# acbull/pyHGT

Measured on AMD Instinct MI355X. Metric: HGTConv forward edges/sec, higher is better.
Workload: dtype f32 (typed linears and relation transforms as 3-term fp16 hi/lo MFMA with power-of-two row scales, fp32 accumulate)

## Files before the change

include/hgt_hip.h:

```cpp
#ifndef HGT_HIP_H_
#define HGT_HIP_H_

#include <stddef.h>
#include <stdint.h>

#ifdef __cplusplus
extern "C" {
#endif

#define HGT_ABI_VERSION 8

#define HGT_OK 0
#define HGT_ERR_INVALID_ARG (-1)
#define HGT_ERR_UNSUPPORTED (-2)
#define HGT_ERR_WORKSPACE (-3)
#define HGT_ERR_TOO_LARGE (-4)
#define HGT_ERR_LAUNCH (-5)

#define HGT_RTE_LEN 240

const char* hgt_strerror(int code);
int hgt_abi_version(void);
#define HGT_FEATURE_LAB_KERNELS 1
#define HGT_FEATURE_DETERMINISTIC_TRAINING 2
// ... 76 lines not shown
                             void* stream);
int hgt_linear_update_f16x3(const float* agg, int64_t ld_agg, const int32_t* rows, const int32_t* group_off,
                            int32_t n_groups, int64_t n_rows, int32_t k, int32_t n_out, const void* w_split,
                            const float* bias, int64_t b_group_stride, const float* x_skip, int64_t ld_skip,
                            const float* skip, const float* ln_w, const float* ln_b, int32_t use_norm, float* out,
                            void* stream);
int hgt_zero_rows(const int32_t* rows, const int32_t* range, int32_t d, float* out, void* stream);

int hgt_relation_pack(const float* relation_att, const float* relation_msg, const float* relation_pri,
                      int32_t n_relations, int32_t n_heads, int32_t n_heads_layout, int32_t d_k, int32_t dk_pad,
                      float* att_t, float* msg_p, void* stream);

int hgt_edge_logits(const void* plan, int64_t n_nodes, int64_t n_edges, int32_t n_types, int32_t n_relations,
                    int32_t n_heads, int32_t dk_pad, const float* Q, const float* K, const float* rte_k,
                    const float* att_t, float* logits, void* stream);
int hgt_edge_logits_mfma(const void* plan, int64_t n_nodes, int64_t n_edges, int32_t n_types, int32_t n_relations,
                         int32_t n_heads, int32_t dk_pad, const float* Q, const float* K, const float* rte_k,
                         const float* att_t, const void* att_frag, int32_t frag_f16, float* logits, void* stream);
int hgt_relation_kside_bytes(int32_t n_relations, int32_t n_heads, int32_t dk_pad, uint64_t* out_host);
int hgt_relation_kside_pack(const float* att_t, int32_t n_relations, int32_t n_heads, int32_t dk_pad, void* att_kside, void* stream);
int hgt_edge_logits_kside(const void* plan, int64_t n_nodes, int64_t n_edges, int32_t n_types, int32_t n_relations,
                          int32_t n_heads, int32_t dk_pad, const float* Q, const float* K, const float* rte_k,
                          const float* att_t, const void* att_kside, int32_t frag_f16, float* logits, void* stream);
int hgt_kside_image_map(int32_t n_blocks, int32_t* image_map, int32_t* b_col, int32_t* c_out);
int hgt_edge_logits_range(const void* plan, int64_t n_nodes, int64_t n_edges, int32_t n_types, int32_t n_relations,
                          int32_t n_heads, int32_t dk_pad, const float* Q, const float* K, const float* rte_k,
                          const float* att_t, const void* att_frag, int32_t frag_f16, float* logits, int32_t item_begin,
                          int32_t item_end, void* stream);
int hgt_edge_softmax(const void* plan, int64_t n_nodes, int64_t n_edges, int32_t n_types, int32_t n_relations,
                     int32_t n_heads, float* logits_att, void* stream);
int hgt_edge_aggregate(const void* plan, int64_t n_nodes, int64_t n_edges, int32_t n_types, int32_t n_relations,
                       int32_t n_heads, int32_t dk_pad, const float* logits, const float* V, const float* rte_v,
                       const float* msg_p, const void* msg_frag, float* agg, int64_t n_q_rows, int32_t apply_gelu,
                       void* hub_ws, void* stream);
int hgt_edge_aggregate_items_bytes(int64_t n_edges, int32_t n_heads, int32_t dk_pad, uint64_t* out_host);
int hgt_edge_aggregate_items(const void* plan, int64_t n_nodes, int64_t n_edges, int32_t n_types, int32_t n_relations,
                             int32_t n_heads, int32_t dk_pad, const float* logits, const float* V, const float* rte_v,
                             const void* msg_frag, int32_t frag_f16, float* agg, int64_t n_q_rows, int32_t apply_gelu,
                             void* scratch, uint64_t scratch_bytes, void* stream);
int hgt_edge_aggregate_items_update(const void* plan, int64_t n_nodes, int64_t n_edges, int32_t n_types, int32_t n_relations,
                                    int32_t n_heads, int32_t dk_pad, const float* logits, const float* V, const float* rte_v,
                                    const void* msg_frag, int32_t frag_f16, int64_t n_q_rows, void* scratch, uint64_t scratch_bytes,
                                    const int32_t* rows, const int32_t* group_off, int32_t n_groups, const void* w_a_split,
                                    const float* b_a, const float* x_skip, int64_t ld_skip, const float* skip, const float* ln_w,
                                    const float* ln_b, int32_t use_norm, int32_t n_out, float* out, void* stream);
int hgt_edge_single_pass_items(const void* plan, int64_t n_nodes, int64_t n_edges, int32_t n_types, int32_t n_relations,
// ... 174 lines not shown
    int32_t stage;
    const int32_t* proj_rows;
    const int32_t* proj_off;
    int64_t proj_n;
    void* prepared;
    uint64_t prepared_bytes;
    int32_t prepared_valid;
    int32_t plan_no_hubs;
    int32_t flags;
    int32_t slice_index;
    int32_t slice_count;
    int64_t q_begin, q_end;
    int32_t item_begin, item_end;
    const void* proj_c24;
    int64_t proj_c24_row0;
} hgt_conv_args;

#define HGT_FLAG_NO_FUSED_UPDATE 1
#define HGT_FLAG_VALU_AGGREGATE  2
#define HGT_FLAG_MFMA_LOGITS     4
#define HGT_FLAG_VALU_LOGITS     8
#define HGT_FLAG_KSIDE_LOGITS 65536
#define HGT_FLAG_NO_KSIDE_LOGITS 131072
#define HGT_FLAG_ITEM_AGGREGATE 16
#define HGT_FLAG_NO_ITEM_AGGREGATE 32
#define HGT_FLAG_FUSED_ANY_SIZE 64
#define HGT_FLAG_SINGLE_PASS 256
#define HGT_FLAG_XS_GEMM_ALWAYS 1024
#define HGT_FLAG_XS_GEMM_NEVER 2048
#define HGT_FLAG_NO_TILE_GEMM 4096
#define HGT_FLAG_NO_MERGE_UPDATE 8192
#define HGT_FLAG_NO_COOP_EDGE 16384
#define HGT_FLAG_COOP_EDGE_ALWAYS 32768
#define HGT_FLAG_RING_AGGREGATE 512
#define HGT_FLAG_DETERMINISTIC_HUBS 128

#define HGT_N_PHASE_EVENTS 7

int hgt_conv_workspace_bytes(int64_t n_nodes, int64_t n_edges, int32_t in_dim, int32_t out_dim,
                             int32_t n_types, int32_t n_relations, int32_t n_heads, int32_t use_rte,
                             uint64_t* out_host);
int hgt_conv_workspace_bytes_ex(int64_t n_nodes, int64_t n_edges, int32_t in_dim, int32_t out_dim,
                                int32_t n_types, int32_t n_relations, int32_t n_heads, int32_t use_rte, int32_t options,
                                uint64_t* out_host);
int hgt_conv_prepared_bytes(int32_t in_dim, int32_t out_dim, int32_t n_types, int32_t n_relations, int32_t n_heads,
                            int32_t use_rte, uint64_t* out_host);
// ... 132 lines not shown
```

pyhgt_amd/_lib.py:

```python
import ctypes as C
import os

_HERE = os.path.dirname(os.path.abspath(__file__))
LIB_PATH = os.environ.get("HGT_LIB_PATH", os.path.join(_HERE, "lib", "libhgt_hip.so"))

HGT_RTE_LEN = 240
HGT_N_PHASE_EVENTS = 7
HGT_FLAG_NO_FUSED_UPDATE = 1
HGT_FLAG_VALU_AGGREGATE = 2
HGT_FLAG_MFMA_LOGITS = 4
HGT_FLAG_VALU_LOGITS = 8
HGT_FLAG_ITEM_AGGREGATE = 16
HGT_FLAG_NO_ITEM_AGGREGATE = 32
HGT_FLAG_FUSED_ANY_SIZE = 64
HGT_FLAG_DETERMINISTIC_HUBS = 128
HGT_FLAG_SINGLE_PASS = 256
HGT_FLAG_RING_AGGREGATE = 512
HGT_FLAG_XS_GEMM_ALWAYS = 1024
HGT_FLAG_XS_GEMM_NEVER = 2048
HGT_FLAG_NO_TILE_GEMM = 4096
HGT_FLAG_NO_MERGE_UPDATE = 8192
HGT_FLAG_NO_COOP_EDGE = 16384
HGT_FLAG_COOP_EDGE_ALWAYS = 32768
HGT_FLAG_KSIDE_LOGITS = 65536
HGT_FLAG_NO_KSIDE_LOGITS = 131072
HGT_LINEAR_FORCE_XS = 0x100
HGT_LINEAR_NO_XS = 0x200
HGT_LINEAR_NO_TILE = 0x400
HGT_LINEAR_TANH = 0x1000
HGT_FEATURE_LAB_KERNELS = 1
HGT_FEATURE_DETERMINISTIC_TRAINING = 2
HGT_STACK_MAX_PIECES = 256
HGT_SAMPLER_MAX_TYPES = 16
HGT_SAMPLER_MAX_TRIPLES = 48
HGT_SAMPLER_MAX_NUMBER = 1024
HGT_SAMPLER_HUB_DEG = 512
HGT_SAMPLER_TIME_NONE = -2 ** 31
HGT_SAMPLER_MAX_BATCH = 64


class HgtLayout(C.Structure):
    _fields_ = [("d_k", C.c_int32), ("dk_pad", C.c_int32), ("d_pad", C.c_int32), ("vec", C.c_int32), ("heads", C.c_int32)]


class HgtPlanSizes(C.Structure):
    _fields_ = [("plan_bytes", C.c_uint64), ("tmp_bytes", C.c_uint64), ("max_items", C.c_int64), ("n_bins", C.c_int64)]


# ... 65 lines not shown
    "hgt_plan_build": (C.c_int, [_vp, _i64, _i64, _vp, _vp, _vp, _i64, _i64, _i64, _i32, _i32, _vp, _u64, _vp, _u64, _vp]),
    "hgt_plan_from_sorted": (C.c_int, [_vp, _vp, _vp, _vp, _vp, _i64, _i64, _i64, _i32, _i32, _vp, _u64, _vp, _u64, _vp]),
    "hgt_typed_linear": (C.c_int, [_vp, _i64, _vp, _vp, _i32, _i64, _i32, _i32, _vp, _i64, _vp, _i64, _vp, _vp, _vp,
                                   _i32, _i32, _i32, _i32, _vp]),
    "hgt_split_weights_bytes": (C.c_int, [_i32, _i32, _i32, C.POINTER(_u64)]),
    "hgt_split_weights": (C.c_int, [_vp, _i64, _i32, _i32, _i32, _vp, _vp]),
    "hgt_typed_linear_bf16x3": (C.c_int, [_vp, _i64, _vp, _vp, _i32, _i64, _i32, _i32, _vp, _vp, _i64, _vp, _vp, _vp,
                                          _i32, _i32, _i32, _vp]),
    "hgt_linear_update_bf16x3": (C.c_int, [_vp, _i64, _vp, _vp, _i32, _i64, _i32, _i32, _vp, _vp, _i64, _vp, _i64, _vp, _vp, _vp,
                                           _i32, _vp, _vp]),
    "hgt_split_weights_f16": (C.c_int, [_vp, _i64, _i32, _i32, _i32, _vp, _vp]),
    "hgt_typed_linear_xs_schedule": (C.c_int, [_vp, _i32, _i64, _i32, _i32, _vp, _i64, C.POINTER(_i64)]),
    "hgt_typed_linear_f16x3": (C.c_int, [_vp, _i64, _vp, _vp, _i32, _i64, _i32, _i32, _vp, _vp, _i64, _vp, _vp, _vp,
                                         _i32, _i32, _i32, _vp]),
    "hgt_linear_update_f16x3": (C.c_int, [_vp, _i64, _vp, _vp, _i32, _i64, _i32, _i32, _vp, _vp, _i64, _vp, _i64, _vp, _vp, _vp,
                                          _i32, _vp, _vp]),
    "hgt_zero_rows": (C.c_int, [_vp, _vp, _i32, _vp, _vp]),
    "hgt_relation_pack": (C.c_int, [_vp, _vp, _vp, _i32, _i32, _i32, _i32, _i32, _vp, _vp, _vp]),
    "hgt_edge_logits": (C.c_int, [_vp, _i64, _i64, _i32, _i32, _i32, _i32, _vp, _vp, _vp, _vp, _vp, _vp]),
    "hgt_edge_logits_mfma": (C.c_int, [_vp, _i64, _i64, _i32, _i32, _i32, _i32, _vp, _vp, _vp, _vp, _vp, _i32, _vp, _vp]),
    "hgt_relation_kside_bytes": (C.c_int, [_i32, _i32, _i32, C.POINTER(_u64)]),
    "hgt_relation_kside_pack": (C.c_int, [_vp, _i32, _i32, _i32, _vp, _vp]),
    "hgt_edge_logits_kside": (C.c_int, [_vp, _i64, _i64, _i32, _i32, _i32, _i32, _vp, _vp, _vp, _vp, _vp, _i32, _vp, _vp]),
    "hgt_kside_image_map": (C.c_int, [_i32, _vp, _vp, _vp]),
    "hgt_edge_logits_range": (C.c_int, [_vp, _i64, _i64, _i32, _i32, _i32, _i32, _vp, _vp, _vp, _vp, _vp, _i32, _vp, _i32, _i32, _vp]),
    "hgt_edge_aggregate_update_range": (C.c_int, [_vp, _i64, _i64, _i32, _i32, _i32, _i32, _vp, _vp, _vp, _vp, _vp, _vp, _i64, _vp, _vp, _vp,
                                                  _vp, _vp, _vp, _i64, _vp, _vp, _vp, _i32, _i32, _vp, _vp, _i64, _i64, _i32, _i32]),
    "hgt_hub_workspace_bytes_ex": (C.c_int, [_i64, _i32, _i32, _i32, _i32, C.POINTER(_u64)]),
    "hgt_edge_aggregate_ex": (C.c_int, [_vp, _i64, _i64, _i32, _i32, _i32, _i32, _vp, _vp, _vp, _vp, _vp, _i32, _vp, _i64, _i32, _vp, _i32, _vp]),
    "hgt_edge_logits_slice": (C.c_int, [_vp, _i64, _i64, _i32, _i32, _i32, _i32, _vp, _vp, _vp, _vp, _vp, _i32, _i32, _vp]),
    "hgt_edge_aggregate_slice": (C.c_int, [_vp, _i64, _i64, _i32, _i32, _i32, _i32, _vp, _vp, _vp, _vp, _vp, _vp, _i64, _i32, _vp,
                                           _i32, _i32, _vp, _i32, _i32, _vp]),
    "hgt_edge_aggregate_slice_ex": (C.c_int, [_vp, _i64, _i64, _i32, _i32, _i32, _i32, _vp, _vp, _vp, _vp, _vp, _vp, _i64, _i32, _vp,
                                              _i32, _i32, _vp, _i32, _i32, _i32, _vp]),
    "hgt_edge_softmax": (C.c_int, [_vp, _i64, _i64, _i32, _i32, _i32, _vp, _vp]),
    "hgt_edge_aggregate": (C.c_int, [_vp, _i64, _i64, _i32, _i32, _i32, _i32, _vp, _vp, _vp, _vp, _vp, _vp, _i64, _i32, _vp, _vp]),
    "hgt_edge_aggregate_f16x3": (C.c_int, [_vp, _i64, _i64, _i32, _i32, _i32, _i32, _vp, _vp, _vp, _vp, _vp, _vp, _i64, _i32, _vp, _vp]),
    "hgt_relation_frag_pack_f16": (C.c_int, [_vp, _i32, _i32, _i32, _vp, _vp]),
    "hgt_edge_aggregate_items_bytes": (C.c_int, [_i64, _i32, _i32, C.POINTER(_u64)]),
    "hgt_edge_spmm_items": (C.c_int, [_vp, _i64, _i64, _i32, _i32, _i32, _i32, _vp, _vp, _vp, _vp, _vp, _i64, _i64, _vp, _u64, _vp]),
    "hgt_edge_aggregate_items_update": (C.c_int, [_vp, _i64, _i64, _i32, _i32, _i32, _i32, _vp, _vp, _vp, _vp, _i32, _i64, _vp, _u64, _vp, _vp, _i32,
                                                  _vp, _vp, _vp, _i64, _vp, _vp, _vp, _i32, _i32, _vp, _vp]),
    "hgt_edge_aggregate_items": (C.c_int, [_vp, _i64, _i64, _i32, _i32, _i32, _i32, _vp, _vp, _vp, _vp, _i32, _vp, _i64, _i32, _vp, _u64, _vp]),
    "hgt_edge_single_pass_items": (C.c_int, [_vp, _i64, _i64, _i32, _i32, _i32, _i32, _vp, _vp, _vp, _vp, _vp, _vp, _vp, _i32, _vp, _i64, _i32,
                                             _vp, _u64, _vp]),
    "hgt_plan_header_to_host": (C.c_int, [_vp, _vp, _vp]),
    "hgt_relation_frag_bytes": (C.c_int, [_i32, _i32, _i32, C.POINTER(_u64)]),
# ... 119 lines not shown
```

pyhgt_amd/csrc/hgt_api.hip:

```cpp
#include "hgt_common.h"

#ifndef HGT_FUSED_MIN_NODES
#define HGT_FUSED_MIN_NODES 16384
#endif
#ifndef HGT_ITEM_AGG_MAX_NODES
#define HGT_ITEM_AGG_MAX_NODES 65536
#endif
#ifndef HGT_ITEM_AGG_DEFAULT_NODES
#define HGT_ITEM_AGG_DEFAULT_NODES 65536
#endif

int hgt_edge_logits_kside_items(const void* plan, int64_t N, int64_t E, int32_t T, int32_t R, int32_t H, int32_t dk_pad, const float* Q,
                                const float* K, const float* rte_k, const void* att_kside, float* logits, int item_lo, int item_hi, void* stream);

namespace {

struct ConvWorkspace {
    uint64_t off_q, off_k, off_v, off_logits, off_agg, off_trans, off_att_t, off_msg_p, off_msg_f, off_att_f, off_att_k, off_hub;
    uint64_t off_rte_lin, off_rte_k, off_rte_v, off_rte_rows, off_rte_off, off_ws_qkv, off_ws_a, off_ws_rte, off_off2, off_pending, off_state, off_zitems, zitems_bytes, total;
    void drop_item_scratch() { zitems_bytes = 0; total = off_zitems; }
};

static ConvWorkspace conv_workspace(int64_t N, int64_t NQ, int64_t E, int in_dim, int out_dim, int T, int R, int , int use_rte,
                                    const hgt_layout& lay, bool item_scratch = true, bool det_hubs = false) {
    const int H = lay.heads;
    ConvWorkspace w;
    uint64_t o = 0;
    auto take = [&](uint64_t bytes) { uint64_t r = o; o = hgt_align_up(o + bytes, 256); return r; };
    const uint64_t dp = (uint64_t)lay.d_pad;
    w.off_q = take((uint64_t)NQ * dp * 4);
    w.off_k = take((uint64_t)N * dp * 4);
    w.off_v = take((uint64_t)N * dp * 4);
    w.off_logits = take((uint64_t)E * H * 4);
    w.off_agg = take((uint64_t)NQ * dp * 4);
    w.off_trans = take((uint64_t)NQ * out_dim * 4);
    w.off_att_t = take((uint64_t)R * H * lay.dk_pad * lay.dk_pad * 4);
// ... 62 lines not shown
    hgt_relation_kside_bytes(R, H, lay.dk_pad, &b);
    p.off_att_k = take(b);
    hgt_split_weights_bytes(T, in_dim, 3 * lay.d_pad, &b);
    p.off_ws_qkv = take(b);
    hgt_split_weights_bytes(T, lay.d_pad, out_dim, &b);
    p.off_ws_upd = take(b);
    p.off_rte_k = take(use_rte ? (uint64_t)T * HGT_RTE_LEN * lay.d_pad * 4 : 0);
    p.off_rte_v = take(use_rte ? (uint64_t)T * HGT_RTE_LEN * lay.d_pad * 4 : 0);
    p.total = o;
    return p;
}

__global__ void k_rte_row_lists(int T, int32_t* __restrict__ rows, int32_t* __restrict__ off) {
    const int i = blockIdx.x * blockDim.x + threadIdx.x;
    if (i < T * HGT_RTE_LEN) rows[i] = i % HGT_RTE_LEN;
    if (i <= T) off[i] = i * HGT_RTE_LEN;
}

enum LogitsForm { LOGITS_VALU, LOGITS_MFMA, LOGITS_SLICE, LOGITS_RANGE, LOGITS_KSIDE };
enum AggForm { AGG_SINGLE_PASS, AGG_FUSED, AGG_ITEMS_UPDATE, AGG_ITEMS, AGG_SLICE, AGG_SUBTILE };
enum UpdateForm { UPDATE_IN_AGGREGATION, UPDATE_LINEAR_FUSED, UPDATE_LINEAR_NODE, UPDATE_DENSE };
struct ConvRoute {
    LogitsForm logits;
    bool kside_range;
    bool mfma_logits;
    AggForm agg[5];
    int n_agg;
    UpdateForm update;
};

struct Conv {
    const hgt_conv_args* a;
    hipStream_t stream;
    hgt_layout lay;
    ConvWorkspace w;
    PreparedLayout pl;
    hgt_plan_rows pr;
    int64_t N, E, NQ;
    int T, R, H, din, dout, dp, dkp, stage, fmode, sl_lo, sl_hi, sl_more;
    bool f16, split, dense, det_hubs, no_unknown_rows, have_frags, have_kside, mfma_agg;
    decltype(&hgt_split_weights) split_weights;
    bool fresh;
    bool wa_prepared;
    char* wb;
    float *Q, *K, *V, *logits, *agg, *trans, *att_t, *msg_p, *rte_k, *rte_v;
    void *msg_f_buf, *att_f_buf, *att_k_buf, *msg_f, *hub_ws, *ws_qkv, *ws_upd, *ws_a;
// ... 71 lines not shown
        att_t = (float*)(pb ? pb + pl.off_att_t : wb + w.off_att_t);
        msg_p = (float*)(pb ? pb + pl.off_msg_p : wb + w.off_msg_p);
        msg_f_buf = pb ? pb + pl.off_msg_f : wb + w.off_msg_f;
        att_f_buf = pb ? pb + pl.off_att_f : wb + w.off_att_f;
        att_k_buf = pb ? pb + pl.off_att_k : wb + w.off_att_k;
        rte_k = a->use_rte ? (float*)(pb ? pb + pl.off_rte_k : wb + w.off_rte_k) : nullptr;
        rte_v = a->use_rte ? (float*)(pb ? pb + pl.off_rte_v : wb + w.off_rte_v) : nullptr;
        ws_qkv = pb ? (void*)(pb + pl.off_ws_qkv) : (void*)(wb + w.off_ws_qkv);
        ws_a = wb + w.off_ws_a;
        wa_prepared = pb && !dense;
        ws_upd = wa_prepared ? (void*)(pb + pl.off_ws_upd) : ws_a;
        msg_f = mfma_agg ? msg_f_buf : nullptr;
    }

    void route() {
        const int fl = a->flags;
        const bool sliced = (stage == 4);
        r.mfma_logits = have_frags && !(fl & HGT_FLAG_VALU_LOGITS) && stage != 4 && (dkp >= 64 || (fl & HGT_FLAG_MFMA_LOGITS));
        r.logits = stage == 5 ? LOGITS_RANGE : sliced ? LOGITS_SLICE : r.mfma_logits ? LOGITS_MFMA : LOGITS_VALU;
        const bool kside_covered = have_kside && split && !a->use_rte && stage != 4 &&
                                   (uint64_t)N * (uint64_t)H * (uint64_t)dkp * 4u < (1ull << 32);
        const bool kside = kside_covered && !(fl & HGT_FLAG_NO_KSIDE_LOGITS) &&
                           ((fl & HGT_FLAG_KSIDE_LOGITS) || (hgt_item_edges(E) >= 64 && !(fl & (HGT_FLAG_MFMA_LOGITS | HGT_FLAG_VALU_LOGITS))));
        r.kside_range = kside && stage == 5;
        if (kside && stage != 5) r.logits = LOGITS_KSIDE;
        const bool fused = split && !dense && dp <= 256 && dout <= dp && (dout & 3) == 0 && (din & 3) == 0 &&
                           (NQ >= HGT_FUSED_MIN_NODES || (fl & HGT_FLAG_FUSED_ANY_SIZE)) &&
                           !(fl & HGT_FLAG_NO_FUSED_UPDATE) && !sliced &&
                           !(f16 && !mfma_agg);
        const bool items = mfma_agg && !sliced && w.zitems_bytes > 0 && NQ < HGT_ITEM_AGG_MAX_NODES && R < 64 &&
                           !(fl & HGT_FLAG_NO_ITEM_AGGREGATE) &&
                           (NQ < HGT_ITEM_AGG_DEFAULT_NODES || (fl & HGT_FLAG_ITEM_AGGREGATE));
        r.n_agg = 0;
        if (items && !fused && !a->want_att && have_frags && E > 0 && (fl & HGT_FLAG_SINGLE_PASS)) r.agg[r.n_agg++] = AGG_SINGLE_PASS;
        if (fused) r.agg[r.n_agg++] = AGG_FUSED;
        if (items && !dense && !(fl & HGT_FLAG_NO_MERGE_UPDATE) && dp <= 512 && dout <= 512 && dout <= dp && (dout & 3) == 0 && (din & 3) == 0)
            r.agg[r.n_agg++] = AGG_ITEMS_UPDATE;
        if (items) r.agg[r.n_agg++] = AGG_ITEMS;
        r.agg[r.n_agg++] = sliced ? AGG_SLICE : AGG_SUBTILE;
        const bool fuse_update = !dense && split && (dout <= 256 || (dout <= 512 && dp <= 512)) && (dout & 3) == 0 && (din & 3) == 0;
        r.update = dense ? UPDATE_DENSE : fuse_update ? UPDATE_LINEAR_FUSED : UPDATE_LINEAR_NODE;
    }

    void mark(int i) const {
        if (a->phase_events && a->phase_events[i]) (void)hipEventRecord((hipEvent_t)a->phase_events[i], stream);
    }
// ... 50 lines not shown
        int rc = linear(a->x, din, pr.rows_q, pr.off_q, T, NQ, din, dp, a->w_qkv, wstride, a->b_qkv, 3 * dp, Q, nullptr, nullptr, dp, 0, ws_a);
        if (rc != HGT_OK) return rc;
        rc = linear(a->x, din, pr.rows_all, pr.off_all, T, N, din, 2 * dp, a->w_qkv + (int64_t)dp * din, wstride, a->b_qkv + dp, 3 * dp,
                    K, V, nullptr, dp, 0, wb + w.off_ws_qkv);
        if (rc != HGT_OK || !(a->prepared && fresh && split)) return rc;
        return split_weights(a->w_qkv, wstride, T, din, 3 * dp, ws_qkv, stream);
    }

    int temporal_tables() const {
        if (!a->use_rte || !fresh) return HGT_OK;
        float* rte_lin = (float*)(wb + w.off_rte_lin);
        int32_t* rrows = (int32_t*)(wb + w.off_rte_rows);
        int32_t* roff = (int32_t*)(wb + w.off_rte_off);
        k_rte_row_lists<<<(T * HGT_RTE_LEN + 255) / 256, 256, 0, stream>>>(T, rrows, roff);
        int rc = linear(a->rte_emb, din, rrows, roff, 1, HGT_RTE_LEN, din, din, a->rte_w, 0, a->rte_b, 0, rte_lin, nullptr, nullptr, din, 1,
                        wb + w.off_ws_rte);
        if (rc != HGT_OK) return rc;
        return linear(rte_lin, din, rrows, roff, T, (int64_t)T * HGT_RTE_LEN, din, 2 * dp, a->w_qkv + (int64_t)dp * din, (int64_t)3 * dp * din,
                      nullptr, 0, rte_k, rte_v, nullptr, dp, 1, ws_a);
    }

    int edge_logits() const {
        if (r.logits == LOGITS_KSIDE) {
            const int rc = hgt_edge_logits_kside(a->plan, N, E, T, R, H, dkp, Q, K, rte_k, att_t, att_k_buf, fmode, logits, stream);
            if (rc != HGT_ERR_UNSUPPORTED) return rc;
            if (r.mfma_logits) return hgt_edge_logits_mfma(a->plan, N, E, T, R, H, dkp, Q, K, rte_k, att_t, att_f_buf, fmode, logits, stream);
        }
        switch (r.logits) {
            case LOGITS_RANGE:
                if (r.kside_range) {
                    const int rc = hgt_edge_logits_kside_items(a->plan, N, E, T, R, H, dkp, Q, K, rte_k, att_k_buf, logits, a->item_begin, a->item_end, stream);
                    if (rc != HGT_ERR_UNSUPPORTED) return rc;
                }
                return hgt_edge_logits_range(a->plan, N, E, T, R, H, dkp, Q, K, rte_k, att_t, r.mfma_logits ? att_f_buf : nullptr, fmode, logits,
                                             a->item_begin, a->item_end, stream);
            case LOGITS_SLICE: return hgt_edge_logits_slice(a->plan, N, E, T, R, H, dkp, Q, K, rte_k, att_t, logits, sl_lo, sl_hi, stream);
            case LOGITS_MFMA: return hgt_edge_logits_mfma(a->plan, N, E, T, R, H, dkp, Q, K, rte_k, att_t, att_f_buf, fmode, logits, stream);
            default: return hgt_edge_logits(a->plan, N, E, T, R, H, dkp, Q, K, rte_k, att_t, logits, stream);
        }
    }

    int aggregate_update(int64_t q0, int64_t q1, int hub_det) const {
        return hgt_edge_aggregate_update_sel(a->plan, N, E, T, R, H, dkp, logits, V, rte_v, msg_p, msg_f, agg, NQ, hub_ws,
                                             (int32_t*)(wb + w.off_pending), a->node_type, ws_upd, a->b_a, a->x, din, a->skip, a->ln_w,
                                             a->ln_b, a->use_norm, dout, a->out, stream, q0, q1, f16 ? 1 : 0, hub_det,
                                             (a->flags & HGT_FLAG_RING_AGGREGATE) ? 1 : 0);
    }

    int aggregate(AggForm form) const {
        void* zitems = wb + w.off_zitems;
        switch (form) {
            case AGG_SINGLE_PASS:
                return hgt_edge_single_pass_items(a->plan, N, E, T, R, H, dkp, Q, K, V, rte_k, rte_v, att_f_buf, msg_f, f16 ? 1 : 0, agg, NQ,
                                                  dense ? 0 : 1, zitems, w.zitems_bytes, stream);
// ... 175 lines not shown
```

pyhgt_amd/csrc/hgt_edge_logits_kside.hip:

```cpp
#include "hgt_edge_common.h"
#include "hgt_split_common.h"
#include "hgt_kside_map.h"

#ifndef HGT_LOGITS_XCD
#define HGT_LOGITS_XCD 1
#endif

namespace {

typedef unsigned hgt_u32x2 __attribute__((ext_vector_type(2)));

__device__ __forceinline__ void half_pair(unsigned x, unsigned& lo, unsigned& up) {
#if __has_builtin(__builtin_amdgcn_permlane32_swap)
    const hgt_u32x2 r = __builtin_amdgcn_permlane32_swap(x, x, false, false);
    lo = r[0];
    up = r[1];
#else
    const unsigned o = (unsigned)__shfl_xor((int)x, 32);
    const bool upper = (threadIdx.x & 32) != 0;
    lo = upper ? o : x;
    up = upper ? x : o;
#endif
}
__device__ __forceinline__ unsigned half_max_bits(unsigned x) {
// ... 49 lines not shown
        unsigned short hi, lo;
        split1_t<true>(v, scale, hi, lo);
        img[hgt_kside_image_index(rh, s, 0, lane, j)] = hi;
        img[hgt_kside_image_index(rh, s, 1, lane, j)] = lo;
    }
    if (t == 0) reinterpret_cast<int*>(img + (int64_t)n_rh * HGT_KSIDE_BLOCK_ELEMS)[rh] = e - 141;
}

struct KsideRows {
    float4 k[4], q[4];
};

typedef unsigned hgt_u32x4 __attribute__((ext_vector_type(4)));
typedef __amdgpu_buffer_rsrc_t kside_rsrc;

__device__ __forceinline__ kside_rsrc kside_table(const float* p, unsigned bytes) {
    return __builtin_amdgcn_make_buffer_rsrc(const_cast<float*>(p), 0, (int)bytes, 0x00020000);
}
__device__ __forceinline__ float4 kside_load16(kside_rsrc t, unsigned off) {
    const hgt_u32x4 v = __builtin_amdgcn_raw_buffer_load_b128(t, (int)off, 0, 0);
    return __builtin_bit_cast(float4, v);
}

template <int H>
__device__ __forceinline__ void kside_issue(kside_rsrc K, kside_rsrc Q, unsigned koff, unsigned qoff, int h, KsideRows& b) {
#pragma unroll
    for (int i = 0; i < 4; ++i) b.k[i] = kside_load16(K, koff + h * 128 + 16 * i);
#pragma unroll
    for (int i = 0; i < 4; ++i) b.q[i] = kside_load16(Q, qoff + h * 128 + 16 * i);
}

__device__ __forceinline__ float kside_head(const KsideRows& b, const hgt_f16x8 (&ah)[2], const hgt_f16x8 (&al)[2], int ea) {
    const int ek = kside_exp(half_max_bits(abs_bits16(b.k)));
    const float ks = kside_scale(ek);
    hgt_f16x8 kh[2], kl[2];
#pragma unroll
    for (int s = 0; s < 2; ++s) {
        static_assert(hgt_kside_k_col(1, 0, 0) == 8 && hgt_kside_k_col(0, 1, 0) == 16, "k-step s takes floats 8 s .. 8 s + 7 of the lane's piece");
        uint4 hi, lo;
        split2_f16(b.k[2 * s].x * ks, b.k[2 * s].y * ks, hi.x, lo.x);
        split2_f16(b.k[2 * s].z * ks, b.k[2 * s].w * ks, hi.y, lo.y);
        split2_f16(b.k[2 * s + 1].x * ks, b.k[2 * s + 1].y * ks, hi.z, lo.z);
        split2_f16(b.k[2 * s + 1].z * ks, b.k[2 * s + 1].w * ks, hi.w, lo.w);
        kh[s] = __builtin_bit_cast(hgt_f16x8, hi);
        kl[s] = __builtin_bit_cast(hgt_f16x8, lo);
    }
    f32x16 acc = {0.f, 0.f, 0.f, 0.f, 0.f, 0.f, 0.f, 0.f, 0.f, 0.f, 0.f, 0.f, 0.f, 0.f, 0.f, 0.f};
    acc = __builtin_amdgcn_mfma_f32_32x32x16_f16(al[0], kh[0], acc, 0, 0, 0);
    acc = __builtin_amdgcn_mfma_f32_32x32x16_f16(al[1], kh[1], acc, 0, 0, 0);
    acc = __builtin_amdgcn_mfma_f32_32x32x16_f16(ah[0], kl[0], acc, 0, 0, 0);
    acc = __builtin_amdgcn_mfma_f32_32x32x16_f16(ah[1], kl[1], acc, 0, 0, 0);
    acc = __builtin_amdgcn_mfma_f32_32x32x16_f16(ah[0], kh[0], acc, 0, 0, 0);
    acc = __builtin_amdgcn_mfma_f32_32x32x16_f16(ah[1], kh[1], acc, 0, 0, 0);
    int eq = (int)(half_max_bits(abs_bits16(b.q)) >> 23);
    eq = eq < 1 ? 1 : (eq > 253 ? 253 : eq);
    const float qs = __builtin_bit_cast(float, (unsigned)(254 - eq) << 23);
    static_assert(hgt_kside_c_out(1, 5) == 21, "register reg of the accumulator is output 16 half + reg: the lane's own Q piece");
    const hgt_f32x2 qs2 = {qs, qs};
    hgt_f32x2 d = {0.0f, 0.0f};
#pragma unroll
    for (int i = 0; i < 4; ++i) {
        const hgt_f32x2 q0 = {b.q[i].x, b.q[i].y}, q1 = {b.q[i].z, b.q[i].w};
        const hgt_f32x2 a0 = {acc[4 * i], acc[4 * i + 1]}, a1 = {acc[4 * i + 2], acc[4 * i + 3]};
        d = __builtin_elementwise_fma(q0 * qs2, a0, d);
        d = __builtin_elementwise_fma(q1 * qs2, a1, d);
    }
    const float d0 = d[0], d1 = d[1];
    return ldexpf(half_sum(d0 + d1), (eq - 127) + (ek - 141) + ea);
}

template <int H>
__global__ __launch_bounds__(256, 2) void k_edge_logits_kside(
    const HgtItem* __restrict__ items, const HgtPlanHeader* __restrict__ hdr, const int32_t* __restrict__ esrc,
    const int32_t* __restrict__ edst, const float* __restrict__ Qp, const float* __restrict__ Kp, unsigned table_bytes,
    const unsigned short* __restrict__ img, float* __restrict__ logits, int R, int item_lo, int item_hi, int items_cap) {
    static_assert(H == 2 || H == 4 || H == 8, "one head group of 32-column heads");
    constexpr int HW = H < 4 ? H : 4, WPI = H / HW;
    constexpr unsigned ROWB = H * 128;
    const int lane = threadIdx.x & 63;
    const int wib = __builtin_amdgcn_readfirstlane(threadIdx.x >> 6);
#if HGT_LOGITS_XCD
    constexpr int XC = 16;
    const int q8 = (int)(blockIdx.x >> 3), vblock = (q8 / XC) * (8 * XC) + (int)(blockIdx.x & 7u) * XC + (q8 % XC);
#else
    const int vblock = blockIdx.x;
#endif
    const int item = item_lo + vblock * (4 / WPI) + wib / WPI;
    const int h0 = (wib % WPI) * HW;
    const HgtItem it = items[min(item, items_cap - 1)];
    if (item >= (item_hi >= 0 ? item_hi : hdr->n_items)) return;
    const int beg = __builtin_amdgcn_readfirstlane(it.beg), end = __builtin_amdgcn_readfirstlane(it.end);
    const int rel = __builtin_amdgcn_readfirstlane(it.rel);
    if (beg >= end) return;
    if (rel >= R) {
        if (h0 == 0)
            for (int64_t i = (int64_t)beg * H + lane; i < (int64_t)end * H; i += 64) logits[i] = 0.0f;
        return;
    }
    const int el = lane & 31, half = lane >> 5;
    const kside_rsrc K = kside_table(Kp, table_bytes), Q = kside_table(Qp, table_bytes);

    hgt_f16x8 ah[HW][2], al[HW][2];
    {
        const uint4* ip = reinterpret_cast<const uint4*>(img) + ((int64_t)rel * H + h0) * 256 + lane;
#pragma unroll
        for (int h = 0; h < HW; ++h)
#pragma unroll
            for (int s = 0; s < 2; ++s) {
                ah[h][s] = __builtin_bit_cast(hgt_f16x8, ip[((h * 2 + s) * 2 + 0) * 64]);
                al[h][s] = __builtin_bit_cast(hgt_f16x8, ip[((h * 2 + s) * 2 + 1) * 64]);
            }
    }
    const int* eap = reinterpret_cast<const int*>(img + (int64_t)R * H * HGT_KSIDE_BLOCK_ELEMS) + rel * H + h0;
    int ea[HW];
#pragma unroll
    for (int h = 0; h < HW; ++h) ea[h] = eap[h];

    const unsigned lo = (unsigned)half * 64u + (unsigned)h0 * 128u;
    int li = min(beg + el, end - 1);
    unsigned koff = (unsigned)esrc[li] * ROWB + lo, qoff = (unsigned)edst[li] * ROWB + lo;
    li = min(beg + 32 + el, end - 1);
    unsigned koff_n = (unsigned)esrc[li] * ROWB + lo, qoff_n = (unsigned)edst[li] * ROWB + lo;
    KsideRows buf[HW];
#pragma unroll
    for (int h = 0; h < HW - 1; ++h) kside_issue<H>(K, Q, koff, qoff, h, buf[h]);
    li = min(beg + 64 + el, end - 1);
    int s2 = esrc[li], d2 = edst[li];
    for (int base = beg; base < end; base += 32) {
        float lg[HW];
#pragma unroll
        for (int h = 0; h < HW; ++h) {
            if (h == 0) kside_issue<H>(K, Q, koff, qoff, HW - 1, buf[HW - 1]);
            else kside_issue<H>(K, Q, koff_n, qoff_n, h - 1, buf[h - 1]);
            __builtin_amdgcn_sched_barrier(0);
            lg[h] = kside_head(buf[h], ah[h], al[h], ea[h]);
            __builtin_amdgcn_sched_barrier(0);
        }
        if (half == 0 && base + el < end) {
            float* o = logits + (int64_t)(base + el) * H + h0;
            if constexpr (HW == 2) *reinterpret_cast<float2*>(o) = make_float2(lg[0], lg[1]);
            else *reinterpret_cast<float4*>(o) = make_float4(lg[0], lg[1], lg[2], lg[3]);
        }
        koff = koff_n;
        qoff = qoff_n;
        koff_n = (unsigned)s2 * ROWB + lo;
        qoff_n = (unsigned)d2 * ROWB + lo;
        li = min(base + 96 + el, end - 1);
        s2 = esrc[li];
        d2 = edst[li];
    }
}

template <int H>
static void launch_kside(const HgtPlanView& pv, const float* Q, const float* K, unsigned table_bytes, const unsigned short* img, float* logits, int R,
                         int item_lo, int item_hi, hipStream_t stream) {
    constexpr int IPW = H == 8 ? 2 : 4;
    const int64_t n_launch = item_hi >= 0 ? (int64_t)(item_hi - item_lo) : pv.L.max_items;
    const unsigned blocks = ((unsigned)((n_launch + IPW - 1) / IPW) + 127u) & ~127u;
    k_edge_logits_kside<H><<<blocks, 256, 0, stream>>>(pv.items, pv.hdr, pv.esrc, pv.edst, Q, K, table_bytes, img, logits, R, item_lo, item_hi, (int)pv.L.max_items);
}

static bool kside_layout(int32_t H, int32_t dk_pad) { return dk_pad == HGT_KSIDE_DK && (H == 2 || H == 4 || H == 8); }

}

extern "C" int hgt_relation_kside_bytes(int32_t R, int32_t H, int32_t dk_pad, uint64_t* out) {
    if (!out || R <= 0 || H <= 0 || dk_pad <= 0) return HGT_ERR_INVALID_ARG;
    *out = kside_layout(H, dk_pad) ? (uint64_t)R * H * HGT_KSIDE_BLOCK_ELEMS * 2 + hgt_align_up((uint64_t)R * H * 4, 256) : 0;
    return HGT_OK;
}

extern "C" int hgt_relation_kside_pack(const float* att_t, int32_t R, int32_t H, int32_t dk_pad, void* att_kside, void* stream) {
    if (!att_t || !att_kside || R <= 0 || H <= 0 || dk_pad <= 0) return HGT_ERR_INVALID_ARG;
    if (!kside_layout(H, dk_pad)) return HGT_ERR_UNSUPPORTED;
    k_relation_kside_pack<<<(unsigned)(R * H), 256, 0, (hipStream_t)stream>>>(att_t, R * H, (unsigned short*)att_kside);
    HGT_CHECK_LAUNCH();
    return HGT_OK;
}

__attribute__((visibility("hidden"))) int hgt_edge_logits_kside_items(const void* plan, int64_t N, int64_t E, int32_t T, int32_t R, int32_t H,
                                                                      int32_t dk_pad, const float* Q, const float* K, const float* rte_k,
                                                                      const void* att_kside, float* logits, int item_lo, int item_hi, void* stream) {
    if (!plan || !Q || !K || !att_kside || (E > 0 && !logits) || N < 0 || E < 0 || R <= 0 || H <= 0 || 64 % H != 0 || dk_pad <= 0)
        return HGT_ERR_INVALID_ARG;
    if (dk_pad % (64 / H) != 0) return HGT_ERR_INVALID_ARG;
    if (!kside_layout(H, dk_pad) || rte_k || (uint64_t)N * (uint64_t)H * (uint64_t)dk_pad * 4u >= (1ull << 32)) return HGT_ERR_UNSUPPORTED;
    if (E == 0) return HGT_OK;
    const HgtPlanView pv = hgt_plan_view(plan, N, E, T, R);
    const unsigned short* img = (const unsigned short*)att_kside;
    const unsigned table_bytes = (unsigned)((uint64_t)N * H * dk_pad * 4u);
    if (H == 2) launch_kside<2>(pv, Q, K, table_bytes, img, logits, R, item_lo, item_hi, (hipStream_t)stream);
    else if (H == 4) launch_kside<4>(pv, Q, K, table_bytes, img, logits, R, item_lo, item_hi, (hipStream_t)stream);
    else launch_kside<8>(pv, Q, K, table_bytes, img, logits, R, item_lo, item_hi, (hipStream_t)stream);
    HGT_CHECK_LAUNCH();
    return HGT_OK;
}

extern "C" int hgt_edge_logits_kside(const void* plan, int64_t N, int64_t E, int32_t T, int32_t R, int32_t H, int32_t dk_pad,
                                     const float* Q, const float* K, const float* rte_k, const float* att_t, const void* att_kside,
                                     int32_t frag_f16, float* logits, void* stream) {
    (void)att_t;
    (void)frag_f16;
    return hgt_edge_logits_kside_items(plan, N, E, T, R, H, dk_pad, Q, K, rte_k, att_kside, logits, 0, -1, stream);
}

extern "C" int hgt_kside_image_map(int32_t n_blocks, int32_t* image_map, int32_t* b_col, int32_t* c_out) {
    if (n_blocks < 0) return HGT_ERR_INVALID_ARG;
    if (image_map)
        for (int64_t rh = 0; rh < n_blocks; ++rh)
            for (int s = 0; s < 2; ++s)
                for (int term = 0; term < 2; ++term)
                    for (int lane = 0; lane < 64; ++lane)
                        for (int j = 0; j < 8; ++j) {
                            int32_t* o = image_map + 4 * hgt_kside_image_index(rh, s, term, lane, j);
                            o[0] = (int32_t)rh, o[1] = term, o[2] = hgt_kside_image_out(lane), o[3] = hgt_kside_image_k(s, lane, j);
                        }
    for (int lane = 0; lane < 64; ++lane) {
        if (b_col)
            for (int s = 0; s < 2; ++s)
                for (int j = 0; j < 8; ++j) b_col[(s * 64 + lane) * 8 + j] = hgt_kside_k_col(s, lane >> 5, j);
        if (c_out)
            for (int reg = 0; reg < 16; ++reg) c_out[lane * 16 + reg] = hgt_kside_c_out(lane >> 5, reg);
    }
    return HGT_OK;
}
```

pyhgt_amd/csrc/hgt_kside_map.h:

```cpp
#pragma once
#include <stdint.h>

#if defined(__HIPCC__) || defined(__CUDACC__)
#define HGT_KSIDE_HD __host__ __device__
#else
#define HGT_KSIDE_HD
#endif

constexpr int HGT_KSIDE_DK = 32;
constexpr int HGT_KSIDE_BLOCK_ELEMS = 2 * 2 * 64 * 8;

HGT_KSIDE_HD constexpr int hgt_kside_row_out(int m) { return 16 * ((m >> 2) & 1) + (m & 3) + 4 * (m >> 3); }
HGT_KSIDE_HD constexpr int hgt_kside_k_col(int s, int half, int j) { return 16 * half + 8 * s + j; }
HGT_KSIDE_HD constexpr int hgt_kside_c_out(int half, int reg) { return hgt_kside_row_out((reg & 3) + 8 * (reg >> 2) + 4 * half); }

HGT_KSIDE_HD constexpr int64_t hgt_kside_image_index(int64_t rh, int s, int term, int lane, int j) {
    return (((rh * 2 + s) * 2 + term) * 64 + lane) * 8 + j;
}
HGT_KSIDE_HD constexpr int hgt_kside_image_out(int lane) { return hgt_kside_row_out(lane & 31); }
HGT_KSIDE_HD constexpr int hgt_kside_image_k(int s, int lane, int j) { return hgt_kside_k_col(s, lane >> 5, j); }

static_assert(hgt_kside_c_out(0, 0) == 0 && hgt_kside_c_out(0, 15) == 15 && hgt_kside_c_out(1, 0) == 16 && hgt_kside_c_out(1, 15) == 31,
              "a lane receives 16 consecutive outputs");
```

Baseline: 1.451 billion.

## Add coalesced-load variant of kside logits kernel with LDS transpose

Adds a second form of the kside edge-logits kernel. Each group of 8 lanes loads one edge's 128-byte row piece (coalesced), and the data is transposed through swizzled LDS to the lane layout the MFMA expects. The default stays the original per-lane gather form, and the coalesced form is chosen only via a new flag. The prefetch of the next edge's indices is also restructured to compute bases one iteration ahead with sched barriers, which touches the default path as well.

```diff
diff --git a/include/hgt_hip.h b/include/hgt_hip.h
--- a/include/hgt_hip.h
+++ b/include/hgt_hip.h
@@ -122,6 +122,12 @@
 int hgt_edge_logits_kside(const void* plan, int64_t n_nodes, int64_t n_edges, int32_t n_types, int32_t n_relations,
                           int32_t n_heads, int32_t dk_pad, const float* Q, const float* K, const float* rte_k,
                           const float* att_t, const void* att_kside, int32_t frag_f16, float* logits, void* stream);
+#define HGT_KSIDE_FORM_COALESCED 0
+#define HGT_KSIDE_FORM_LANE_GATHER 1
+int hgt_edge_logits_kside_form(const void* plan, int64_t n_nodes, int64_t n_edges, int32_t n_types, int32_t n_relations,
+                               int32_t n_heads, int32_t dk_pad, const float* Q, const float* K, const float* rte_k,
+                               const float* att_t, const void* att_kside, int32_t frag_f16, float* logits, int32_t form, void* stream);
+int hgt_kside_gather_map(int32_t* load_map, int32_t* read_off);
 int hgt_kside_image_map(int32_t n_blocks, int32_t* image_map, int32_t* b_col, int32_t* c_out);
 int hgt_edge_logits_range(const void* plan, int64_t n_nodes, int64_t n_edges, int32_t n_types, int32_t n_relations,
                           int32_t n_heads, int32_t dk_pad, const float* Q, const float* K, const float* rte_k,
@@ -342,6 +348,7 @@
 #define HGT_FLAG_VALU_LOGITS     8
 #define HGT_FLAG_KSIDE_LOGITS 65536
 #define HGT_FLAG_NO_KSIDE_LOGITS 131072
+#define HGT_FLAG_KSIDE_COALESCED 262144
 #define HGT_FLAG_ITEM_AGGREGATE 16
 #define HGT_FLAG_NO_ITEM_AGGREGATE 32
 #define HGT_FLAG_FUSED_ANY_SIZE 64
diff --git a/pyhgt_amd/_lib.py b/pyhgt_amd/_lib.py
--- a/pyhgt_amd/_lib.py
+++ b/pyhgt_amd/_lib.py
@@ -24,6 +24,9 @@
 HGT_FLAG_COOP_EDGE_ALWAYS = 32768
 HGT_FLAG_KSIDE_LOGITS = 65536
 HGT_FLAG_NO_KSIDE_LOGITS = 131072
+HGT_FLAG_KSIDE_COALESCED = 262144
+HGT_KSIDE_FORM_COALESCED = 0
+HGT_KSIDE_FORM_LANE_GATHER = 1
 HGT_LINEAR_FORCE_XS = 0x100
 HGT_LINEAR_NO_XS = 0x200
 HGT_LINEAR_NO_TILE = 0x400
@@ -135,7 +138,9 @@
     "hgt_relation_kside_bytes": (C.c_int, [_i32, _i32, _i32, C.POINTER(_u64)]),
     "hgt_relation_kside_pack": (C.c_int, [_vp, _i32, _i32, _i32, _vp, _vp]),
     "hgt_edge_logits_kside": (C.c_int, [_vp, _i64, _i64, _i32, _i32, _i32, _i32, _vp, _vp, _vp, _vp, _vp, _i32, _vp, _vp]),
+    "hgt_edge_logits_kside_form": (C.c_int, [_vp, _i64, _i64, _i32, _i32, _i32, _i32, _vp, _vp, _vp, _vp, _vp, _i32, _vp, _i32, _vp]),
     "hgt_kside_image_map": (C.c_int, [_i32, _vp, _vp, _vp]),
+    "hgt_kside_gather_map": (C.c_int, [_vp, _vp]),
     "hgt_edge_logits_range": (C.c_int, [_vp, _i64, _i64, _i32, _i32, _i32, _i32, _vp, _vp, _vp, _vp, _vp, _i32, _vp, _i32, _i32, _vp]),
     "hgt_edge_aggregate_update_range": (C.c_int, [_vp, _i64, _i64, _i32, _i32, _i32, _i32, _vp, _vp, _vp, _vp, _vp, _vp, _i64, _vp, _vp, _vp,
                                                   _vp, _vp, _vp, _i64, _vp, _vp, _vp, _i32, _i32, _vp, _vp, _i64, _i64, _i32, _i32]),
diff --git a/pyhgt_amd/csrc/hgt_api.hip b/pyhgt_amd/csrc/hgt_api.hip
--- a/pyhgt_amd/csrc/hgt_api.hip
+++ b/pyhgt_amd/csrc/hgt_api.hip
@@ -11,7 +11,7 @@
 #endif
 
 int hgt_edge_logits_kside_items(const void* plan, int64_t N, int64_t E, int32_t T, int32_t R, int32_t H, int32_t dk_pad, const float* Q,
-                                const float* K, const float* rte_k, const void* att_kside, float* logits, int item_lo, int item_hi, void* stream);
+                                const float* K, const float* rte_k, const void* att_kside, float* logits, int item_lo, int item_hi, int form, void* stream);
 
 namespace {
 
@@ -120,6 +120,7 @@
 enum UpdateForm { UPDATE_IN_AGGREGATION, UPDATE_LINEAR_FUSED, UPDATE_LINEAR_NODE, UPDATE_DENSE };
 struct ConvRoute {
     LogitsForm logits;
+    int kside_form;
     bool kside_range;
     bool mfma_logits;
     AggForm agg[5];
@@ -237,6 +238,7 @@
                                    (uint64_t)N * (uint64_t)H * (uint64_t)dkp * 4u < (1ull << 32);
         const bool kside = kside_covered && !(fl & HGT_FLAG_NO_KSIDE_LOGITS) &&
                            ((fl & HGT_FLAG_KSIDE_LOGITS) || (hgt_item_edges(E) >= 64 && !(fl & (HGT_FLAG_MFMA_LOGITS | HGT_FLAG_VALU_LOGITS))));
+        r.kside_form = (fl & HGT_FLAG_KSIDE_COALESCED) ? HGT_KSIDE_FORM_COALESCED : HGT_KSIDE_FORM_LANE_GATHER;
         r.kside_range = kside && stage == 5;
         if (kside && stage != 5) r.logits = LOGITS_KSIDE;
         const bool fused = split && !dense && dp <= 256 && dout <= dp && (dout & 3) == 0 && (din & 3) == 0 &&
@@ -333,14 +335,15 @@
 
     int edge_logits() const {
         if (r.logits == LOGITS_KSIDE) {
-            const int rc = hgt_edge_logits_kside(a->plan, N, E, T, R, H, dkp, Q, K, rte_k, att_t, att_k_buf, fmode, logits, stream);
+            const int rc = hgt_edge_logits_kside_form(a->plan, N, E, T, R, H, dkp, Q, K, rte_k, att_t, att_k_buf, fmode, logits, r.kside_form, stream);
             if (rc != HGT_ERR_UNSUPPORTED) return rc;
             if (r.mfma_logits) return hgt_edge_logits_mfma(a->plan, N, E, T, R, H, dkp, Q, K, rte_k, att_t, att_f_buf, fmode, logits, stream);
         }
         switch (r.logits) {
             case LOGITS_RANGE:
                 if (r.kside_range) {
-                    const int rc = hgt_edge_logits_kside_items(a->plan, N, E, T, R, H, dkp, Q, K, rte_k, att_k_buf, logits, a->item_begin, a->item_end, stream);
+                    const int rc = hgt_edge_logits_kside_items(a->plan, N, E, T, R, H, dkp, Q, K, rte_k, att_k_buf, logits, a->item_begin, a->item_end, r.kside_form,
+                                                               stream);
                     if (rc != HGT_ERR_UNSUPPORTED) return rc;
                 }
                 return hgt_edge_logits_range(a->plan, N, E, T, R, H, dkp, Q, K, rte_k, att_t, r.mfma_logits ? att_f_buf : nullptr, fmode, logits,
diff --git a/pyhgt_amd/csrc/hgt_edge_logits_kside.hip b/pyhgt_amd/csrc/hgt_edge_logits_kside.hip
--- a/pyhgt_amd/csrc/hgt_edge_logits_kside.hip
+++ b/pyhgt_amd/csrc/hgt_edge_logits_kside.hip
@@ -95,12 +95,57 @@
     return __builtin_bit_cast(float4, v);
 }
 
-template <int H>
-__device__ __forceinline__ void kside_issue(kside_rsrc K, kside_rsrc Q, unsigned koff, unsigned qoff, int h, KsideRows& b) {
-#pragma unroll
-    for (int i = 0; i < 4; ++i) b.k[i] = kside_load16(K, koff + h * 128 + 16 * i);
-#pragma unroll
-    for (int i = 0; i < 4; ++i) b.q[i] = kside_load16(Q, qoff + h * 128 + 16 * i);
+__device__ __forceinline__ int kside_in_loop(int x) {
+    asm volatile("" : "+v"(x));
+    return x;
+}
+
+template <bool LANE_GATHER>
+struct KsideBases {
+    unsigned k[LANE_GATHER ? 1 : 4], q[LANE_GATHER ? 1 : 4];
+};
+template <bool LANE_GATHER>
+__device__ __forceinline__ void kside_bases(unsigned krow, unsigned qrow, int lane, KsideBases<LANE_GATHER>& b) {
+    if constexpr (LANE_GATHER) {
+        b.k[0] = krow + (unsigned)(lane >> 5) * 64u;
+        b.q[0] = qrow + (unsigned)(lane >> 5) * 64u;
+    } else {
+        const unsigned piece = (unsigned)hgt_kside_gather_piece(lane) * 16u;
+        static_assert(hgt_kside_gather_edge(3, 9) == hgt_kside_gather_edge(0, 9) + 24, "load j reads from lane 8 j + the lane of load 0");
+        const int from = kside_in_loop(hgt_kside_gather_edge(0, lane) * 4);
+#pragma unroll
+        for (int j = 0; j < 4; ++j) {
+            b.k[j] = (unsigned)__builtin_amdgcn_ds_bpermute(from + 32 * j, (int)krow) + piece;
+            b.q[j] = (unsigned)__builtin_amdgcn_ds_bpermute(from + 32 * j, (int)qrow) + piece;
+        }
+    }
+}
+
+template <bool LANE_GATHER>
+__device__ __forceinline__ void kside_issue(kside_rsrc K, kside_rsrc Q, const KsideBases<LANE_GATHER>& a, int h, KsideRows& b) {
+#pragma unroll
+    for (int i = 0; i < 4; ++i) b.k[i] = kside_load16(K, (LANE_GATHER ? a.k[0] + 16 * i : a.k[i]) + h * 128);
+#pragma unroll
+    for (int i = 0; i < 4; ++i) b.q[i] = kside_load16(Q, (LANE_GATHER ? a.q[0] + 16 * i : a.q[i]) + h * 128);
+}
+
+__device__ __forceinline__ void kside_wave_sync() {
+    __builtin_amdgcn_fence(__ATOMIC_RELEASE, "wavefront");
+    __builtin_amdgcn_wave_barrier();
+    __builtin_amdgcn_fence(__ATOMIC_ACQUIRE, "wavefront");
+}
+__device__ __forceinline__ void kside_transpose(char* slot, unsigned wr0, unsigned rd0, KsideRows& b) {
+    const unsigned wr = (unsigned)kside_in_loop((int)wr0), rd = (unsigned)kside_in_loop((int)rd0);
+#pragma unroll
+    for (int j = 0; j < 4; ++j) *reinterpret_cast<float4*>(slot + ((wr ^ (64u * (j & 1))) + 1024u * j)) = b.k[j];
+#pragma unroll
+    for (int j = 0; j < 4; ++j) *reinterpret_cast<float4*>(slot + HGT_KSIDE_LINE_IMAGE_BYTES + ((wr ^ (64u * (j & 1))) + 1024u * j)) = b.q[j];
+    kside_wave_sync();
+#pragma unroll
+    for (int i = 0; i < 4; ++i) b.k[i] = *reinterpret_cast<const float4*>(slot + (rd ^ (16u * i)));
+#pragma unroll
+    for (int i = 0; i < 4; ++i) b.q[i] = *reinterpret_cast<const float4*>(slot + HGT_KSIDE_LINE_IMAGE_BYTES + (rd ^ (16u * i)));
+    kside_wave_sync();
 }
 
 __device__ __forceinline__ float kside_head(const KsideRows& b, const hgt_f16x8 (&ah)[2], const hgt_f16x8 (&al)[2], int ea) {
@@ -142,7 +187,7 @@
     return ldexpf(half_sum(d0 + d1), (eq - 127) + (ek - 141) + ea);
 }
 
-template <int H>
+template <int H, bool LANE_GATHER>
 __global__ __launch_bounds__(256, 2) void k_edge_logits_kside(
     const HgtItem* __restrict__ items, const HgtPlanHeader* __restrict__ hdr, const int32_t* __restrict__ esrc,
     const int32_t* __restrict__ edst, const float* __restrict__ Qp, const float* __restrict__ Kp, unsigned table_bytes,
@@ -189,23 +234,42 @@
 #pragma unroll
     for (int h = 0; h < HW; ++h) ea[h] = eap[h];
 
-    const unsigned lo = (unsigned)half * 64u + (unsigned)h0 * 128u;
+    constexpr int SLOT = 2 * HGT_KSIDE_LINE_IMAGE_BYTES;
+    char* slots = nullptr;
+    if constexpr (!LANE_GATHER) {
+        __shared__ __attribute__((aligned(128))) char s_lines[4][2][SLOT];
+        slots = s_lines[wib][0];
+    }
+    const unsigned wr = (unsigned)hgt_kside_lds_write(0, lane), rd = (unsigned)hgt_kside_lds_read(lane, 0);
+    const unsigned lo = (unsigned)h0 * 128u;
     int li = min(beg + el, end - 1);
-    unsigned koff = (unsigned)esrc[li] * ROWB + lo, qoff = (unsigned)edst[li] * ROWB + lo;
+    KsideBases<LANE_GATHER> at;
+    kside_bases<LANE_GATHER>((unsigned)esrc[li] * ROWB + lo, (unsigned)edst[li] * ROWB + lo, lane, at);
     li = min(beg + 32 + el, end - 1);
-    unsigned koff_n = (unsigned)esrc[li] * ROWB + lo, qoff_n = (unsigned)edst[li] * ROWB + lo;
+    int sn = esrc[li], dn = edst[li];
+    __builtin_amdgcn_sched_barrier(0);
     KsideRows buf[HW];
 #pragma unroll
-    for (int h = 0; h < HW - 1; ++h) kside_issue<H>(K, Q, koff, qoff, h, buf[h]);
-    li = min(beg + 64 + el, end - 1);
-    int s2 = esrc[li], d2 = edst[li];
+    for (int h = 0; h < HW - 1; ++h) {
+        kside_issue<LANE_GATHER>(K, Q, at, h, buf[h]);
+        __builtin_amdgcn_sched_barrier(0);
+    }
     for (int base = beg; base < end; base += 32) {
         float lg[HW];
 #pragma unroll
         for (int h = 0; h < HW; ++h) {
-            if (h == 0) kside_issue<H>(K, Q, koff, qoff, HW - 1, buf[HW - 1]);
-            else kside_issue<H>(K, Q, koff_n, qoff_n, h - 1, buf[h - 1]);
+            kside_issue<LANE_GATHER>(K, Q, at, h == 0 ? HW - 1 : h - 1, buf[h == 0 ? HW - 1 : h - 1]);
+            if (h == 0) {
+                kside_bases<LANE_GATHER>((unsigned)sn * ROWB + lo, (unsigned)dn * ROWB + lo, lane, at);
+                li = min(base + 64 + el, end - 1);
+                sn = esrc[li];
+                dn = edst[li];
+            }
             __builtin_amdgcn_sched_barrier(0);
+            if constexpr (!LANE_GATHER) {
+                kside_transpose(slots + (h & 1) * SLOT, wr, rd, buf[h]);
+                __builtin_amdgcn_sched_barrier(0);
+            }
             lg[h] = kside_head(buf[h], ah[h], al[h], ea[h]);
             __builtin_amdgcn_sched_barrier(0);
         }
@@ -214,23 +278,17 @@
             if constexpr (HW == 2) *reinterpret_cast<float2*>(o) = make_float2(lg[0], lg[1]);
             else *reinterpret_cast<float4*>(o) = make_float4(lg[0], lg[1], lg[2], lg[3]);
         }
-        koff = koff_n;
-        qoff = qoff_n;
-        koff_n = (unsigned)s2 * ROWB + lo;
-        qoff_n = (unsigned)d2 * ROWB + lo;
-        li = min(base + 96 + el, end - 1);
-        s2 = esrc[li];
-        d2 = edst[li];
     }
 }
 
 template <int H>
 static void launch_kside(const HgtPlanView& pv, const float* Q, const float* K, unsigned table_bytes, const unsigned short* img, float* logits, int R,
-                         int item_lo, int item_hi, hipStream_t stream) {
+                         int item_lo, int item_hi, int form, hipStream_t stream) {
     constexpr int IPW = H == 8 ? 2 : 4;
     const int64_t n_launch = item_hi >= 0 ? (int64_t)(item_hi - item_lo) : pv.L.max_items;
     const unsigned blocks = ((unsigned)((n_launch + IPW - 1) / IPW) + 127u) & ~127u;
-    k_edge_logits_kside<H><<<blocks, 256, 0, stream>>>(pv.items, pv.hdr, pv.esrc, pv.edst, Q, K, table_bytes, img, logits, R, item_lo, item_hi, (int)pv.L.max_items);
+    auto kernel = form == HGT_KSIDE_FORM_COALESCED ? k_edge_logits_kside<H, false> : k_edge_logits_kside<H, true>;
+    kernel<<<blocks, 256, 0, stream>>>(pv.items, pv.hdr, pv.esrc, pv.edst, Q, K, table_bytes, img, logits, R, item_lo, item_hi, (int)pv.L.max_items);
 }
 
 static bool kside_layout(int32_t H, int32_t dk_pad) { return dk_pad == HGT_KSIDE_DK && (H == 2 || H == 4 || H == 8); }
@@ -253,28 +311,35 @@
 
 __attribute__((visibility("hidden"))) int hgt_edge_logits_kside_items(const void* plan, int64_t N, int64_t E, int32_t T, int32_t R, int32_t H,
                                                                       int32_t dk_pad, const float* Q, const float* K, const float* rte_k,
-                                                                      const void* att_kside, float* logits, int item_lo, int item_hi, void* stream) {
+                                                                      const void* att_kside, float* logits, int item_lo, int item_hi, int form,
+                                                                      void* stream) {
     if (!plan || !Q || !K || !att_kside || (E > 0 && !logits) || N < 0 || E < 0 || R <= 0 || H <= 0 || 64 % H != 0 || dk_pad <= 0)
         return HGT_ERR_INVALID_ARG;
-    if (dk_pad % (64 / H) != 0) return HGT_ERR_INVALID_ARG;
+    if (dk_pad % (64 / H) != 0 || (form != HGT_KSIDE_FORM_COALESCED && form != HGT_KSIDE_FORM_LANE_GATHER)) return HGT_ERR_INVALID_ARG;
     if (!kside_layout(H, dk_pad) || rte_k || (uint64_t)N * (uint64_t)H * (uint64_t)dk_pad * 4u >= (1ull << 32)) return HGT_ERR_UNSUPPORTED;
     if (E == 0) return HGT_OK;
     const HgtPlanView pv = hgt_plan_view(plan, N, E, T, R);
     const unsigned short* img = (const unsigned short*)att_kside;
     const unsigned table_bytes = (unsigned)((uint64_t)N * H * dk_pad * 4u);
-    if (H == 2) launch_kside<2>(pv, Q, K, table_bytes, img, logits, R, item_lo, item_hi, (hipStream_t)stream);
-    else if (H == 4) launch_kside<4>(pv, Q, K, table_bytes, img, logits, R, item_lo, item_hi, (hipStream_t)stream);
-    else launch_kside<8>(pv, Q, K, table_bytes, img, logits, R, item_lo, item_hi, (hipStream_t)stream);
+    if (H == 2) launch_kside<2>(pv, Q, K, table_bytes, img, logits, R, item_lo, item_hi, form, (hipStream_t)stream);
+    else if (H == 4) launch_kside<4>(pv, Q, K, table_bytes, img, logits, R, item_lo, item_hi, form, (hipStream_t)stream);
+    else launch_kside<8>(pv, Q, K, table_bytes, img, logits, R, item_lo, item_hi, form, (hipStream_t)stream);
     HGT_CHECK_LAUNCH();
     return HGT_OK;
+}
+
+extern "C" int hgt_edge_logits_kside_form(const void* plan, int64_t N, int64_t E, int32_t T, int32_t R, int32_t H, int32_t dk_pad,
+                                          const float* Q, const float* K, const float* rte_k, const float* att_t, const void* att_kside,
+                                          int32_t frag_f16, float* logits, int32_t form, void* stream) {
+    (void)att_t;
+    (void)frag_f16;
+    return hgt_edge_logits_kside_items(plan, N, E, T, R, H, dk_pad, Q, K, rte_k, att_kside, logits, 0, -1, form, stream);
 }
 
 extern "C" int hgt_edge_logits_kside(const void* plan, int64_t N, int64_t E, int32_t T, int32_t R, int32_t H, int32_t dk_pad,
                                      const float* Q, const float* K, const float* rte_k, const float* att_t, const void* att_kside,
                                      int32_t frag_f16, float* logits, void* stream) {
-    (void)att_t;
-    (void)frag_f16;
-    return hgt_edge_logits_kside_items(plan, N, E, T, R, H, dk_pad, Q, K, rte_k, att_kside, logits, 0, -1, stream);
+    return hgt_edge_logits_kside_form(plan, N, E, T, R, H, dk_pad, Q, K, rte_k, att_t, att_kside, frag_f16, logits, HGT_KSIDE_FORM_LANE_GATHER, stream);
 }
 
 extern "C" int hgt_kside_image_map(int32_t n_blocks, int32_t* image_map, int32_t* b_col, int32_t* c_out) {
@@ -297,3 +362,15 @@
     }
     return HGT_OK;
 }
+
+extern "C" int hgt_kside_gather_map(int32_t* load_map, int32_t* read_off) {
+    for (int lane = 0; lane < 64; ++lane)
+        for (int j = 0; j < 4; ++j) {
+            if (load_map) {
+                int32_t* o = load_map + 3 * (j * 64 + lane);
+                o[0] = hgt_kside_gather_edge(j, lane), o[1] = hgt_kside_gather_piece(lane), o[2] = hgt_kside_lds_write(j, lane);
+            }
+            if (read_off) read_off[lane * 4 + j] = hgt_kside_lds_read(lane, j);
+        }
+    return HGT_OK;
+}
diff --git a/pyhgt_amd/csrc/hgt_kside_map.h b/pyhgt_amd/csrc/hgt_kside_map.h
--- a/pyhgt_amd/csrc/hgt_kside_map.h
+++ b/pyhgt_amd/csrc/hgt_kside_map.h
@@ -22,3 +22,20 @@
 
 static_assert(hgt_kside_c_out(0, 0) == 0 && hgt_kside_c_out(0, 15) == 15 && hgt_kside_c_out(1, 0) == 16 && hgt_kside_c_out(1, 15) == 31,
               "a lane receives 16 consecutive outputs");
+
+constexpr int HGT_KSIDE_LINE_IMAGE_BYTES = 32 * 128;
+HGT_KSIDE_HD constexpr int hgt_kside_gather_edge(int j, int lane) { return 8 * j + (lane >> 3); }
+HGT_KSIDE_HD constexpr int hgt_kside_gather_piece(int lane) { return lane & 7; }
+HGT_KSIDE_HD constexpr int hgt_kside_lds_cell(int e, int p) { return e * 128 + ((p ^ ((e >> 1) & 7)) * 16); }
+HGT_KSIDE_HD constexpr int hgt_kside_lds_write(int j, int lane) { return hgt_kside_lds_cell(hgt_kside_gather_edge(j, lane), hgt_kside_gather_piece(lane)); }
+HGT_KSIDE_HD constexpr int hgt_kside_lds_read(int lane, int i) { return hgt_kside_lds_cell(lane & 31, 4 * (lane >> 5) + i); }
+
+HGT_KSIDE_HD constexpr bool hgt_kside_lds_addresses_fold() {
+    for (int lane = 0; lane < 64; ++lane)
+        for (int j = 0; j < 4; ++j) {
+            if (hgt_kside_lds_write(j, lane) != (hgt_kside_lds_write(0, lane) ^ (64 * (j & 1))) + 1024 * j) return false;
+            if (hgt_kside_lds_read(lane, j) != (hgt_kside_lds_read(lane, 0) ^ (16 * j))) return false;
+        }
+    return true;
+}
+static_assert(hgt_kside_lds_addresses_fold(), "the LDS addresses of the four writes / reads differ by constants");
```

Result: no change. 1.462 billion (median of 6 runs) (+0.8%).
